# UniBwTAS/continuous_clustering

Measured on AMD Instinct MI355X. Metric: Mpoints/s clustered (64-beam streams), higher is better.
Workload: dtype f32

## Files before the change

continuous_clustering_amd/csrc/cc_device.h:

```cpp
#pragma once
#include <stdint.h>
#include <hip/hip_runtime.h>

#include "../../include/cc_hip.h"

namespace ccd
{

constexpr int WAVE = 64;
constexpr int MAX_ROWS_PER_LANE = 2;
constexpr int LINK_SLOTS = 4;
constexpr int WIN_COLS = 32;
constexpr int PP_SKIP = 0x7fffffff;
#ifndef CC_INS_WIN
#define CC_INS_WIN 64
#endif
constexpr int INS_WIN = CC_INS_WIN;
constexpr int SG_NAN = 1, SG_FOG = 2, SG_EGO = 4, SG_INCL_IGNORE = 8, SG_TOO_CLOSE = 16, SG_PENDING = 32;
constexpr unsigned NAN_RANGE_BITS = 0x7fc00001u;
#ifndef CC_TREE_SLOTS
#define CC_TREE_SLOTS 256
#endif
constexpr int TREE_SLOTS = CC_TREE_SLOTS;
#ifndef CC_TABLE_WAVES
// ... 27 lines not shown
    double finish_lower_bound;
    double last_round_min_az;
    int64_t clear_allowed;
    struct BatchDesc
    {
        int64_t seg_begin;
        int64_t seg_end;
        int64_t acp_next;
        int64_t pub_begin;
        int64_t pub_end;
        int64_t mode;
        int64_t fused;
    } batch[4];
    int32_t assoc_mode;
    int32_t pad1;
    int64_t cursor;
    int64_t pre_seg_begin;
    uint64_t firings_consumed;
    uint64_t cells_published;
    uint64_t clusters_finished;
    uint64_t exceed_one_rotation;
    uint64_t serial_columns;
    uint64_t stamp_alias_rounds;
    uint64_t batch_columns;
    uint64_t batch_bails;
    uint64_t batch_bail_reason[8];
    int64_t par_clear_done;
    int32_t par_bad;
    int32_t par_upto;
    int64_t serial_until;
    uint64_t dbg[16];
    int32_t error;
    int32_t n_events;
    int64_t error_a;
    int64_t error_b;
    int32_t n_links;
    int32_t pad2;
    int64_t overrun_col;
};

struct Planes
{
    float* dist;
    float* incaz;
    uint16_t* gtag;
    uint32_t* src;
    uint8_t* inten;
    int32_t* trig;
    int64_t* colg;
    double* colminaz;
    uint8_t* ground;
    uint8_t* debug;
    uint8_t* ignored;
    int32_t* root;
    uint32_t* id;
    double* t_fin;
    uint32_t* t_width;
    uint32_t* t_pts;
    int32_t* t_uf;
    uint32_t* t_cid;
    int32_t* t_pos;
    uint8_t* t_finished;
    int32_t* ulist;
    int32_t* ucomp;
    unsigned long long* agg_fin;
    long long* agg_min;
    long long* agg_max;
    uint32_t* agg_pts;
    uint32_t* agg_cid;
    int32_t* agg_first;
    uint8_t* agg_flag;
    cc_event* events;
    float* pp_x;
    float* pp_y;
    float* pp_z;
    float* pp_dist;
    float* pp_incl;
    float* pp_incaz;
    int32_t* pp_cir;
    float* sg_x2;
    float* sg_uz;
    uint8_t* sg_flags;
    float* sg_w;
    float4* sc_rec;
    int16_t* sc_parent;
    int16_t* sc_term;
    double* col_newfin;
    int32_t* col_info;
    unsigned* pk_meta;
    double* pk_fin;
    unsigned long long* pk_lk;
    uint16_t* col_act;
    uint8_t* sc_nlinks;
    unsigned long long* sc_links;
    double* sc_fin;
    uint16_t* sc_visits;
    int2* link_log;
    void* sl_rec;
    int32_t* sl_ctl;
    int32_t* sl_cols;
    int32_t* par_off;
    float* curtab;
    unsigned long long* tab_acc;
    float* tabc;
};

// ... 25 lines not shown
```

continuous_clustering_amd/csrc/cc_engine.hip:

```cpp
#include <hip/hip_runtime.h>

#include <algorithm>
#include <chrono>
#include <cstdlib>
#include <cmath>
#include <cstdio>
#include <cstring>
#include <functional>
#include <limits>
#include <mutex>
#include <string>
#include <vector>

#include "cc_kernels.h"

#ifndef CC_LWAVE_MAX_STREAMS
#define CC_LWAVE_MAX_STREAMS 256
#endif

using namespace ccd;

struct cc_engine
{
    int device{0};
// ... 263 lines not shown
    e->d_gather = nullptr;
    e->gather_bytes = 0;
    e->d_take_cursor = nullptr;
    e->d_take_plan = nullptr;
    e->d_take_ctl = nullptr;
    e->d_take_counts = nullptr;
    e->take_counts_cap = 0;
    e->d_tc_cursor = nullptr;
    e->d_tc_plan = nullptr;
    e->d_tc_table = nullptr;
    e->d_tc_ctl = nullptr;
    e->d_tc_slots = nullptr;
    e->tc_slots_cap = 0;
    e->d_small = nullptr;
    e->d_small_seq = nullptr;
    e->d_input_sum = nullptr;
    e->small_view_ok = false;
    e->small_seq_expected = 0;
    free_pinned(e, PIN_SHAPE);
    return CC_OK;
}

int allocate(cc_engine* e)
{
    const Geometry& g = e->g;
    const size_t S = (size_t) g.num_streams;
    const size_t C = S * (size_t) g.cells;
    const size_t L = S * (size_t) g.ring_cols;
    const size_t T = S * (size_t) g.tree_capacity;
    Planes& P = e->P;
    int rc = CC_OK;
    e->slab_planning = getenv("CC_NO_SLAB") == nullptr;
    e->slab_bytes = 0;
    e->slab_plan.clear();
#define A(field, count)                                \
    if ((rc = alloc_plane(e, &P.field, (count))) != 0) \
        return rc;
    A(dist, C) A(incaz, C) A(gtag, C) A(src, C) A(inten, C);
    A(trig, L) A(colg, L) A(colminaz, L);
    A(ground, C) A(debug, C) A(ignored, C) A(root, C) A(id, C);
    A(t_fin, C) A(t_width, C) A(t_pts, C) A(t_uf, C) A(t_cid, C) A(t_pos, C) A(t_finished, C);
    A(ulist, T) A(ucomp, T) A(agg_fin, T) A(agg_min, T) A(agg_max, T) A(agg_pts, T) A(agg_cid, T) A(agg_first, T) A(agg_flag, T);
    A(events, S * (size_t) g.event_capacity);
    A(sc_parent, C) A(sc_nlinks, C) A(sc_links, C) A(sc_fin, C);
    A(sc_term, C) A(col_newfin, L) A(col_info, L) A(col_act, L) A(pk_meta, C) A(pk_fin, C) A(pk_lk, C);
    A(sg_x2, C) A(sg_uz, C) A(sg_w, C) A(sg_flags, C) A(sc_rec, C);
    A(curtab, S * (size_t) g.num_rows);
    A(tab_acc, S * (size_t) g.tab_tiles * (size_t) g.num_rows);
    A(par_off, S * (size_t) cck::IP_MAXF);
    A(tabc, (size_t) BATCH_SLOTS * S * (size_t) g.tab_tiles * (size_t) g.num_rows);
    A(sc_visits, C);
    A(link_log, S * (size_t) g.link_capacity);
    A(sl_ctl, S * 4) A(sl_cols, L);
    if ((rc = alloc_plane(e, (unsigned long long**) &P.sl_rec, S * (size_t) cck::SL_CAP * sizeof(cck::ScanLongRec) / sizeof(unsigned long long))) != 0)
        return rc;
#undef A
    if ((rc = alloc_plane(e, &e->d_states, S)) != 0)
        return rc;
    if ((rc = alloc_plane(e, &e->d_par_left, 16)) != 0)
        return rc;
    if ((rc = alloc_plane(e, &e->d_bail_count, 4)) != 0)
        return rc;
    if ((rc = alloc_plane(e, &e->d_remaining, 1)) != 0)
        return rc;
    const bool slab = e->slab_planning;
    if (e->slab_planning)
    {
        e->slab_planning = false;
        char* base = nullptr;
        if ((rc = alloc_plane(e, &base, e->slab_bytes)) != 0)
            return rc;
        for (auto& f : e->slab_plan)
            *f.first = base + f.second;
        e->slab_plan.clear();
    }
    (void) slab;
    CC_HIP_CHECK(e, hipMemset(e->d_bail_count, 0, 4 * sizeof(int)));
    CC_HIP_CHECK(e, hipMemset(e->d_par_left, 0, 16 * sizeof(int)));
    CC_HIP_CHECK(e, hipMemset(e->d_remaining, 0, sizeof(int)));
    return CC_OK;
}

void fresh_stream_state(const cc_engine* e, StreamState* out)
{
    StreamState& st = *out;
    memset(&st, 0, sizeof(st));
    st.prev_rearmost = 0;
    st.prev_foremost = -1;
    st.first_unfinished = -1;
    st.ring_start = -1;
    st.ring_end = -1;
    st.first_column = -1;
    st.clear_done = -1;
    st.first_unpublished = -1;
    st.cluster_counter = 1;
    st.min_required = 0;
    st.finish_lower_bound = std::numeric_limits<double>::max();
    st.last_round_min_az = -1.0;
    st.overrun_col = std::numeric_limits<int64_t>::max();
    st.n_links = 0;
    for (auto& d : st.batch)
        d.seg_begin = d.seg_end = d.acp_next = d.pub_begin = d.pub_end = -1, d.mode = 0, d.fused = 0;
    st.assoc_mode = e->cfg.max_steps_in_row > WIN_COLS - 2 ? 1 : 0;
}

int reset_state(cc_engine* e, bool keep_table)
{
    e->small_view_ok = false;
    e->widest_steps_in_row = e->cfg.max_steps_in_row;
    std::fill(e->state_cached.begin(), e->state_cached.end(), 0);
    const Geometry& g = e->g;
    const size_t S = (size_t) g.num_streams;
    const size_t C = S * (size_t) g.cells;
    Planes& P = e->P;
    CC_HIP_CHECK(e, hipMemsetAsync(P.dist, 0xFF, C * sizeof(float), e->stream));
    CC_HIP_CHECK(e, hipMemsetAsync(P.gtag, 0, C * sizeof(uint16_t), e->stream));
    CC_HIP_CHECK(e, hipMemsetAsync(P.id, 0, C * sizeof(uint32_t), e->stream));
    CC_HIP_CHECK(e, hipMemsetAsync(P.ground, CC_GP_UNKNOWN, C, e->stream));
    CC_HIP_CHECK(e, hipMemsetAsync(P.debug, CC_DBG_WHITE, C, e->stream));
    CC_HIP_CHECK(e, hipMemsetAsync(P.ignored, 0, C, e->stream));
    CC_HIP_CHECK(e, hipMemsetAsync(P.root, 0xFF, C * sizeof(int32_t), e->stream));
    CC_HIP_CHECK(e, hipMemsetAsync(P.tab_acc, 0, S * (size_t) g.tab_tiles * (size_t) g.num_rows * sizeof(unsigned long long), e->stream));
    CC_HIP_CHECK(e, hipMemsetAsync(P.sl_ctl, 0, S * 4 * sizeof(int32_t), e->stream));
    if (!keep_table)
        CC_HIP_CHECK(e, hipMemsetAsync(P.curtab, 0xFF, S * (size_t) g.num_rows * sizeof(float), e->stream));
    std::vector<StreamState> init(S);
    for (auto& st : init)
        fresh_stream_state(e, &st);
    CC_HIP_CHECK(e, hipMemcpyAsync(e->d_states, init.data(), S * sizeof(StreamState), hipMemcpyHostToDevice, e->stream));
    if (e->d_take_cursor)
        CC_HIP_CHECK(e, hipMemsetAsync(e->d_take_cursor, 0, 2 * S * sizeof(long long), e->stream));
    if (e->d_tc_cursor)
        CC_HIP_CHECK(e, hipMemsetAsync(e->d_tc_cursor, 0, 2 * S * sizeof(long long), e->stream));
    CC_HIP_CHECK(e, hipStreamSynchronize(e->stream));
    for (auto& v : e->pending_events)
        v.clear();
    for (auto& v : e->pending_links)
        v.clear();
    e->batch_open = false;
    for (bool& b : e->assoc_pending)
        b = false;
    e->deferred_tail = nullptr;
    e->lazy_pending = false;
    e->lazy_prev_left = nullptr;
    e->lazy_miss = 0;
    e->lazy_clean = 0;
    e->lazy_ok = true;
    return CC_OK;
}

int reset_streams_state(cc_engine* e, const std::vector<int>& list)
{
    const Geometry& g = e->g;
    const Planes& P = e->P;
    const unsigned long long cells = (unsigned long long) g.cells;
    cck::ResetJob job;
    memset(&job, 0, sizeof(job));
    const cck::ResetFill fills[cck::RESET_PLANES] = {
        {(char*) P.dist, cells * sizeof(float), 0xFF, 0},
        {(char*) P.gtag, cells * sizeof(uint16_t), 0, 0},
        {(char*) P.id, cells * sizeof(uint32_t), 0, 0},
        {(char*) P.ground, cells, CC_GP_UNKNOWN, 0},
        {(char*) P.debug, cells, CC_DBG_WHITE, 0},
        {(char*) P.ignored, cells, 0, 0},
        {(char*) P.root, cells * sizeof(int32_t), 0xFF, 0},
        {(char*) P.tab_acc, (unsigned long long) g.tab_tiles * (unsigned long long) g.num_rows * sizeof(unsigned long long), 0, 0},
        {(char*) P.sl_ctl, 4 * sizeof(int32_t), 0, 0},
    };
    unsigned long long longest = 0;
    for (int k = 0; k < cck::RESET_PLANES; k++)
    {
        job.fill[k] = fills[k];
        longest = std::max(longest, fills[k].bytes);
    }
    fresh_stream_state(e, &job.fresh);
    job.states = e->d_states;
    job.take_cursor = e->d_take_cursor;
    job.tc_cursor = e->d_tc_cursor;
    job.num_streams = g.num_streams;
    int rc = ensure_gather(e, list.size() * sizeof(int));
    if (rc)
        return rc;
    CC_HIP_CHECK(e, hipMemcpyAsync(e->d_gather, list.data(), list.size() * sizeof(int), hipMemcpyHostToDevice, e->stream));
    constexpr size_t MAX_GRID_Y = 65535;
    for (size_t first = 0; first < list.size(); first += MAX_GRID_Y)
    {
        const size_t rows = std::min(MAX_GRID_Y, list.size() - first);
        const unsigned long long want = (longest + cck::RESET_CHUNK_BYTES - 1) / cck::RESET_CHUNK_BYTES;
        const unsigned chunks = (unsigned) std::max<unsigned long long>(1, std::min<unsigned long long>(want, (unsigned long long) cck::RESET_MAX_BLOCKS / rows));
        hipLaunchKernelGGL(cck::k_reset_streams, dim3(chunks, (unsigned) rows), dim3(cck::RESET_THREADS), 0, e->stream, job, (const int*) e->d_gather + first);
    }
    CC_HIP_CHECK(e, hipGetLastError());
    CC_HIP_CHECK(e, hipStreamSynchronize(e->stream));
    for (int s : list)
    {
        e->state_cached[s] = 0;
        if (s == e->small_view_stream)
            e->small_view_ok = false;
        e->pending_events[s].clear();
        e->pending_links[s].clear();
    }
    return CC_OK;
}

int ensure_prep(cc_engine* e, size_t points)
{
    if (e->prep_capacity >= points)
        return CC_OK;
    int rc;
    for (auto& q : e->pp)
        if ((rc = alloc_plane(e, &q.x, points)) || (rc = alloc_plane(e, &q.y, points)) || (rc = alloc_plane(e, &q.z, points)) ||
            (rc = alloc_plane(e, &q.dist, points)) || (rc = alloc_plane(e, &q.incl, points)) ||
            (rc = alloc_plane(e, &q.incaz, points)) || (rc = alloc_plane(e, &q.cir, points)))
            return rc;
    e->prep_capacity = points;
    e->small_graphs_stale = true;
    return CC_OK;
// ... 1949 lines not shown
```

continuous_clustering_amd/csrc/cc_k_base.h:

```cpp
#pragma once

#define CC_PI_F 3.14159274101257324219f
#define CC_2PI_D 6.283185307179586

__device__ __forceinline__ int lane_id()
{
    return threadIdx.x & 63;
}

__device__ __forceinline__ int f2i_x86(float v)
{
    if (!(v > -2147483904.0f && v < 2147483648.0f))
        return (int) 0x80000000;
    return (int) v;
}

template<int CTRL, int ROW_MASK>
__device__ __forceinline__ int dpp_mov_i32(int fill, int v)
{
    return __builtin_amdgcn_update_dpp(fill, v, CTRL, ROW_MASK, 0xf, false);
}
template<int CTRL, int ROW_MASK>
__device__ __forceinline__ long long dpp_mov_i64(long long fill, long long v)
{
// ... 257 lines not shown
}

constexpr uint16_t CELL_CLEARED = 0;
__device__ __forceinline__ uint16_t cell_tag(const long long pass)
{
    return (uint16_t) (0x8000u | ((unsigned) pass & 0x7fffu));
}

constexpr int IP_MAXF = 4608;

struct SP
{
    float *dist, *tabc;
    float* incaz;
    uint16_t* gtag;
    uint32_t* src;
    uint8_t *inten, *ground, *debug, *ignored;
    int32_t* trig;
    int64_t* colg;
    double* colminaz;
    int32_t* root;
    uint32_t* id;
    double* t_fin;
    uint32_t *t_width, *t_pts, *t_cid;
    int32_t *t_uf, *t_pos;
    uint8_t* t_finished;
    int32_t *ulist, *ucomp;
    unsigned long long* agg_fin;
    long long *agg_min, *agg_max;
    uint32_t *agg_pts, *agg_cid;
    int32_t* agg_first;
    uint8_t* agg_flag;
    float* curtab;
    unsigned long long* tab_acc;
    int32_t* par_off;
    cc_event* events;
    int16_t* sc_parent;
    int16_t* sc_term;
    double* col_newfin;
    int32_t* col_info;
    uint16_t* col_act;
    unsigned* pk_meta;
    double* pk_fin;
    unsigned long long* pk_lk;
    uint8_t* sc_nlinks;
    unsigned long long* sc_links;
    double* sc_fin;
    float *sg_x2, *sg_uz, *sg_w;
    uint8_t* sg_flags;
    float4* sc_rec;
    uint16_t* sc_visits;
    int2* link_log;
    int32_t* sl_cols;
};

__device__ __forceinline__ SP stream_ptrs(const Planes& P, const Geometry& g, int s)
{
    SP p;
    const size_t co = (size_t) s * (size_t) g.cells;
    const size_t lo = (size_t) s * (size_t) g.ring_cols;
    const size_t to = (size_t) s * (size_t) g.tree_capacity;
    p.dist = P.dist + co;
    p.incaz = P.incaz + co;
    p.gtag = P.gtag + co;
    p.src = P.src + co;
    p.inten = P.inten + co;
    p.ground = P.ground + co;
    p.debug = P.debug + co;
    p.ignored = P.ignored + co;
    p.trig = P.trig + lo;
    p.colg = P.colg + lo;
    p.colminaz = P.colminaz + lo;
    p.root = P.root + co;
    p.id = P.id + co;
    p.t_fin = P.t_fin + co;
    p.t_width = P.t_width + co;
    p.t_pts = P.t_pts + co;
    p.t_cid = P.t_cid + co;
    p.t_uf = P.t_uf + co;
    p.t_pos = P.t_pos + co;
    p.t_finished = P.t_finished + co;
    p.ulist = P.ulist + to;
    p.ucomp = P.ucomp + to;
    p.agg_fin = P.agg_fin + to;
    p.agg_min = P.agg_min + to;
    p.agg_max = P.agg_max + to;
    p.agg_pts = P.agg_pts + to;
    p.agg_cid = P.agg_cid + to;
    p.agg_first = P.agg_first + to;
    p.agg_flag = P.agg_flag + to;
    p.curtab = P.curtab + (size_t) s * g.num_rows;
    p.par_off = P.par_off + (size_t) s * IP_MAXF;
    p.tab_acc = P.tab_acc + (size_t) s * (size_t) g.tab_tiles * g.num_rows;
    p.tabc = P.tabc + (size_t) s * (size_t) g.tab_tiles * g.num_rows;
    p.events = P.events + (size_t) s * g.event_capacity;
    p.sc_parent = P.sc_parent + co;
    p.sc_term = P.sc_term + co;
    p.col_newfin = P.col_newfin + lo;
    p.col_info = P.col_info + lo;
    p.col_act = P.col_act + lo;
    p.pk_meta = P.pk_meta + co;
    p.pk_fin = P.pk_fin + co;
    p.pk_lk = P.pk_lk + co;
    p.sc_nlinks = P.sc_nlinks + co;
    p.sc_links = P.sc_links + co;
    p.sc_fin = P.sc_fin + co;
    p.sg_x2 = P.sg_x2 + co;
    p.sg_uz = P.sg_uz + co;
    p.sg_w = P.sg_w + co;
    p.sg_flags = P.sg_flags + co;
    p.sc_rec = P.sc_rec + co;
    p.sc_visits = P.sc_visits + co;
    p.link_log = P.link_log + (size_t) s * (size_t) g.link_capacity;
    p.sl_cols = P.sl_cols + lo;
    return p;
}

__device__ __forceinline__ double cell_fin(const cc_config& cfg, const SP& p, const int ci, const CazBase& cb)
{
    if (p.ignored[ci])
        return 0.;
    const float mad = ccm::asinf_exact(cfg.max_distance / p.dist[ci]);
    return cell_caz(cb, p.incaz[ci]) + (double) mad;
}
__device__ __forceinline__ double cell_fin_of(const Geometry& g, const cc_config& cfg, const SP& p, const int ci, const CazBase& cb)
{
    return g.scan_stores_fin ? p.sc_fin[ci] : cell_fin(cfg, p, ci, cb);
}
```

continuous_clustering_amd/csrc/cc_k_reset.h:

```cpp
#pragma once

constexpr int RESET_PLANES = 9;
constexpr int RESET_THREADS = 256;
constexpr unsigned long long RESET_CHUNK_BYTES = 16384;
constexpr int RESET_MAX_BLOCKS = 2048;
static_assert(sizeof(StreamState) % sizeof(unsigned long long) == 0 && alignof(StreamState) == alignof(unsigned long long), "the state is copied in 8-byte words");

struct ResetFill
{
    char* plane;
    unsigned long long bytes;
    unsigned value;
    unsigned pad;
};

struct ResetJob
{
    ResetFill fill[RESET_PLANES];
    StreamState fresh;
    StreamState* states;
    long long* take_cursor;
    long long* tc_cursor;
    int num_streams;
    int pad;
};

__device__ __forceinline__ void fill_slice(char* p, const unsigned long long bytes, const unsigned value, const unsigned chunk, const unsigned chunks)
{
    const unsigned long long to_boundary = (16ull - ((unsigned long long) p & 15ull)) & 15ull;
    const unsigned long long head = to_boundary < bytes ? to_boundary : bytes;
    const unsigned long long words = (bytes - head) >> 4;
    const unsigned long long tail = bytes - head - (words << 4);
    const unsigned w = (value & 0xffu) * 0x01010101u;
    const uint4 v = make_uint4(w, w, w, w);
    uint4* mid = (uint4*) (p + head);
    for (unsigned long long i = (unsigned long long) chunk * RESET_THREADS + threadIdx.x; i < words; i += (unsigned long long) chunks * RESET_THREADS)
        mid[i] = v;
    if (chunk == 0 && threadIdx.x < head)
        p[threadIdx.x] = (char) value;
    if (chunk == chunks - 1 && threadIdx.x < tail)
        p[head + (words << 4) + threadIdx.x] = (char) value;
}

__global__ __launch_bounds__(RESET_THREADS) void k_reset_streams(const ResetJob job, const int* __restrict__ list)
{
    const int s = list[blockIdx.y];
    if (s < 0 || s >= job.num_streams)
        return;
    for (int k = 0; k < RESET_PLANES; k++)
        fill_slice(job.fill[k].plane + (unsigned long long) s * job.fill[k].bytes, job.fill[k].bytes, job.fill[k].value, blockIdx.x, gridDim.x);
    if (blockIdx.x != 0)
        return;
    const unsigned long long* src = (const unsigned long long*) &job.fresh;
    unsigned long long* dst = (unsigned long long*) &job.states[s];
    for (unsigned i = threadIdx.x; i < sizeof(StreamState) / sizeof(unsigned long long); i += RESET_THREADS)
// ... 10 lines not shown
```

continuous_clustering_amd/csrc/cc_k_scan.h:

```cpp
#pragma once

#ifndef CC_SCAN_BLOCKS
#define CC_SCAN_BLOCKS 256
#endif
constexpr int SCAN_BLOCKS = CC_SCAN_BLOCKS;

template<int RPL, bool MIRROR>
__device__ __forceinline__ void scan_body(const Geometry& g, const cc_config& cfg, const Planes& P, StreamState* states, int first_stream, int slot,
                                          const int bx, const int by, const int ny)
{
    const int s = first_stream + bx;
    const int lane = lane_id();
    const StreamState* st = &states[s];
    if (st->error != 0 || st->batch[slot].seg_begin < 0 || st->batch[slot].mode != 0)
        return;
    AssocCtx c;
    c.p = stream_ptrs(P, g, s);
    const SP& p = c.p;
    const int R = c.R = g.num_rows;
    c.NC = g.num_columns;
    const int RC = c.RC = g.ring_cols;
    c.az_width = g.az_width;
    c.maxd2 = g.max_distance_squared;
    c.max_steps_in_row = cfg.max_steps_in_row;
// ... 294 lines not shown
            continue;
        P.pp_x[i] = q.x;
        P.pp_y[i] = q.y;
        P.pp_z[i] = q.z;
        P.pp_dist[i] = q.dist;
        P.pp_incl[i] = q.incl;
        P.pp_incaz[i] = q.incaz;
    }
    if (threadIdx.x == 0)
    {
        long long* w = insert2_sync_words<1>(R);
        lds_st(w, 0ll);
        lds_st(w + 1, 0ll);
        lds_st(w + 2, -1ll);
    }
    __syncthreads();
    SF_MARK(1)
    if (threadIdx.x < 128)
        insert2_body<1, true, true>(g, cfg, P, states, stream, slot, inten, n, remaining, n, 0, 0);
    __syncthreads();
    SF_MARK(2)
    if (threadIdx.x < 64)
        seg_small_body(g, cfg, P, states, stream, slot, poses, n, 0, ego, n, 0);
    __syncthreads();
    SF_MARK(3)
    if (g.mirror_fields)
        scan_body<1, true>(g, cfg, P, states, stream, slot, 0, uniform_i32((int) (threadIdx.x >> 6)), 4);
    else
        scan_body<1, false>(g, cfg, P, states, stream, slot, 0, uniform_i32((int) (threadIdx.x >> 6)), 4);
#ifdef CC_SF_STATS
    __syncthreads();
    SF_MARK(4)
    if (threadIdx.x == 0)
    {
        for (int i = 0; i < 4; i++)
            st->dbg[i] += sf_t[i + 1] - sf_t[i];
        st->dbg[4] += 1;
    }
#endif
}

#ifndef CC_SCAN_TILE_CELLS
#define CC_SCAN_TILE_CELLS 256
#endif
constexpr int SCAN_TILE_CELLS = CC_SCAN_TILE_CELLS;

struct ScanCfg
{
    int R, RC, max_col_steps, stop_min;
    bool stop_enabled;
    float maxd2;
};

struct ScanPoint
{
    float4 me;
    float mad;
    int row, needed, bound;
    int sb, down, d, oc, orow;
    int rooted, parent, nlinks, overflow, visits, reach;
    unsigned long long packed;
    bool run;

    __device__ __forceinline__ void next_column(const ScanCfg& c)
    {
        if ((rooted && c.stop_enabled && sb >= c.stop_min) || oc == bound || sb + 1 > needed)
            run = false;
        else
        {
            sb++;
            oc = oc == 0 ? c.RC - 1 : oc - 1;
            down = 0;
            d = 0;
            orow = row;
        }
    }
    __device__ __forceinline__ void next_direction(const ScanCfg& c)
    {
        if (down == 0 && sb > 0)
        {
            down = 1;
            d = 1;
            orow = row + 1;
            if (!(orow < c.R && d <= c.max_col_steps))
                next_column(c);
        }
        else
            next_column(c);
    }
    __device__ __forceinline__ void start(const ScanCfg& c, const bool have, const int lc)
    {
        sb = 0, down = 0, d = 1, oc = lc, orow = row - 1;
        rooted = 0, parent = -1, nlinks = 0, overflow = 0, visits = 0, reach = 0;
        packed = 0;
        run = have;
        if (run && !(orow >= 0 && d <= c.max_col_steps))
            next_direction(c);
    }
    template<bool MIRROR>
    __device__ __forceinline__ void step(const ScanCfg& c, const SP& p)
    {
        const float4 o = p.sc_rec[oc * c.R + orow];
        const unsigned char oign = p.ignored[oc * c.R + orow];
        if (MIRROR)
        {
            visits++;
            reach = sb;
        }
        if (ccm::absf(o.w - me.w) > mad)
            next_direction(c);
        else
        {
            const float dx = me.x - o.x, dy = me.y - o.y, dz = me.z - o.z;
            if (!oign && dx * dx + dy * dy + dz * dz < c.maxd2)
            {
                const int cand = (sb << 8) | orow;
                if (!rooted)
                    parent = cand;
                else if (nlinks < LINK_SLOTS)
                {
                    packed |= (unsigned long long) cand << (16 * nlinks);
                    nlinks++;
                }
                else
                    overflow = 1;
                rooted = 1;
            }
            if (rooted && c.stop_enabled && d >= c.stop_min)
                next_direction(c);
            else
            {
                d++;
                orow = down ? orow + 1 : orow - 1;
                if (!(orow >= 0 && orow < c.R && d <= c.max_col_steps))
                    next_direction(c);
            }
        }
    }
};

constexpr int SL_CAP = 8192;
struct ScanLongRec
{
    int ci;
    int oc;
    short orow, sb, d, needed;
    short parent;
    unsigned char down, rooted, nlinks, flags;
    float mad;
    unsigned long long packed;
};
static_assert(sizeof(ScanLongRec) == 40, "long-scan record");

#ifndef CC_SCAN_CAP
#define CC_SCAN_CAP 6
#endif
constexpr int SCAN_CAP = CC_SCAN_CAP;

template<int RPL, bool MIRROR, bool SPLIT = false>
__global__ __launch_bounds__(64) void k_scan2(Geometry g, cc_config cfg, Planes P, StreamState* states, int first_stream, int slot)
{
    static_assert(!(SPLIT && MIRROR), "the long-scan list does not carry the mirror's visit counts");
    const int s = first_stream + blockIdx.x;
    const int lane = lane_id();
    const StreamState* st = &states[s];
    if (st->error != 0 || st->batch[slot].seg_begin < 0 || st->batch[slot].mode != 0)
        return;
    const SP p = stream_ptrs(P, g, s);
    const int R = g.num_rows, RC = g.ring_cols;
    ScanCfg sc;
    sc.R = R, sc.RC = RC;
    sc.maxd2 = g.max_distance_squared;
    sc.max_col_steps = cfg.max_steps_in_column;
    sc.stop_enabled = cfg.stop_after_association_enabled != 0;
    sc.stop_min = cfg.stop_after_association_min_steps;
    const int max_row_steps = cfg.max_steps_in_row;
    const int TC = SCAN_TILE_CELLS / (RPL * 64);
    __shared__ unsigned short s_list[SCAN_TILE_CELLS];
    __shared__ short s_parent[SCAN_TILE_CELLS];
    __shared__ unsigned char s_nlinks[SCAN_TILE_CELLS];
    __shared__ unsigned short s_visits[MIRROR ? SCAN_TILE_CELLS : 1];
    __shared__ unsigned char s_reach[MIRROR ? SCAN_TILE_CELLS : 1];
    __shared__ double s_fin[SCAN_TILE_CELLS];
    __shared__ unsigned long long s_links[SCAN_TILE_CELLS];
    int* const sl_ctl = P.sl_ctl + (size_t) s * 4;
    ScanLongRec* const sl_rec = (ScanLongRec*) P.sl_rec + (size_t) s * SL_CAP;
    const long long col_begin = st->batch[slot].acp_next, col_end = st->batch[slot].seg_end, first_column = st->first_column;
    const int first_lc = (int) (first_column % RC);
    const long long n_tiles = (col_end - col_begin + TC - 1) / TC;
    for (long long tile = blockIdx.y; tile < n_tiles; tile += gridDim.y)
    {
        const long long gc0 = col_begin + tile * TC;
        const int ncols = (int) (col_end - gc0 < TC ? col_end - gc0 : TC);
        const int lc0 = (int) (gc0 % RC);
        const long long rot0 = gc0 / g.num_columns;
        const int cir0 = (int) (gc0 - rot0 * g.num_columns);
        int n_act = 0;
        for (int j = 0; j < TC * RPL; j++)
        {
            const int tc = j / RPL, row = (j % RPL) * 64 + lane;
            const int tl = tc * RPL * 64 + row;
            bool act = false;
            if (tc < ncols && row < R)
            {
                int lc = lc0 + tc;
                lc = lc >= RC ? lc - RC : lc;
                act = p.ignored[lc * R + row] == 0;
            }
            s_parent[tl] = -2;
            s_nlinks[tl] = 0;
            s_fin[tl] = 0.;
            s_links[tl] = 0;
            if (MIRROR)
            {
                s_visits[tl] = 0;
                s_reach[tl] = 0;
            }
            const unsigned long long m = __ballot(act);
            if (act)
                s_list[n_act + __popcll(m & lanes_below())] = (unsigned short) tl;
            n_act += __popcll(m);
        }
        wave_lds_fence();
        unsigned deferred = 0;
        for (int base = 0; base < n_act; base += 64)
        {
            const bool have = base + lane < n_act;
            const int tl = have ? (int) s_list[base + lane] : 0;
            const int tc = tl / (RPL * 64), row = tl % (RPL * 64);
            const long long gc = gc0 + tc;
            int lc = lc0 + tc;
            lc = lc >= RC ? lc - RC : lc;
            const int ci = lc * R + row;
            ScanPoint q;
            q.me = make_float4(0.f, 0.f, 0.f, 0.f);
            q.mad = 0.f;
            q.row = row;
            double fin = 0.;
            q.needed = -1;
            if (have)
            {
                q.me = p.sc_rec[ci];
                q.mad = ccm::asinf_exact(cfg.max_distance / p.dist[ci]);
                fin = cell_caz(caz_base_of_rotation(rot0 + (cir0 + tc >= g.num_columns ? 1 : 0)), p.incaz[ci]) + (double) q.mad;
                q.needed = f2i_x86(__builtin_ceilf(q.mad / g.az_width));
                q.needed = q.needed < max_row_steps ? q.needed : max_row_steps;
            }
            q.bound = (gc - first_column) <= (long long) max_row_steps + 1 ? first_lc : -1;
            q.start(sc, have, lc);
            bool pending = false;
            if (SPLIT)
            {
                for (int it = 0; it < g.scan_cap && __any(q.run); it++)
                    if (q.run)
                        q.template step<false>(sc, p);
                const unsigned long long m = __ballot(q.run);
                if (m)
                {
                    int lbase = 0;
                    if (lane == (int) __ffsll((long long) m) - 1)
                        lbase = atomicAdd(&sl_ctl[0], (int) __popcll(m));
                    lbase = __shfl(lbase, (int) __ffsll((long long) m) - 1);
                    const int idx = lbase + (int) __popcll(m & lanes_below());
                    if (q.run && idx < g.sl_cap)
                    {
                        ScanLongRec r;
                        r.ci = ci, r.oc = q.oc;
                        r.orow = (short) q.orow, r.sb = (short) q.sb, r.d = (short) q.d, r.needed = (short) q.needed;
                        r.parent = (short) q.parent;
                        r.down = (unsigned char) q.down, r.rooted = (unsigned char) q.rooted, r.nlinks = (unsigned char) q.nlinks;
                        r.flags = (unsigned char) ((q.overflow ? 1 : 0) | (q.bound >= 0 ? 2 : 0));
                        r.mad = q.mad;
                        r.packed = q.packed;
                        sl_rec[idx] = r;
                        pending = true;
                        q.run = false;
                    }
                    while (__any(q.run))
                        if (q.run)
                            q.template step<false>(sc, p);
                }
                for (int t2 = 0; t2 < TC; t2++)
                    if (__any(pending && tc == t2))
                        deferred |= 1u << t2;
            }
            else
            {
                while (__any(q.run))
                    if (q.run)
                        q.template step<MIRROR>(sc, p);
            }
            if (have)
            {
                s_parent[tl] = (short) (pending ? -3 : q.parent);
                s_nlinks[tl] = (unsigned char) (q.overflow ? 255 : q.nlinks);
                s_fin[tl] = fin;
                s_links[tl] = q.packed;
                if (MIRROR)
                {
                    s_visits[tl] = sat_u16(q.visits);
                    s_reach[tl] = (unsigned char) q.reach;
                }
            }
        }
        wave_lds_fence();
        for (int tc = 0; tc < ncols; tc++)
        {
            int lc = lc0 + tc;
            lc = lc >= RC ? lc - RC : lc;
            int parent[RPL], nlinks[RPL];
            double fin[RPL];
            unsigned long long packed[RPL];
            int reach = 0;
            const bool later = SPLIT && ((deferred >> tc) & 1u) != 0;
#pragma unroll
            for (int k = 0; k < RPL; k++)
            {
                const int row = k * 64 + lane;
                const int tl = tc * RPL * 64 + row;
                parent[k] = s_parent[tl];
                nlinks[k] = s_nlinks[tl];
                fin[k] = s_fin[tl];
                packed[k] = s_links[tl];
                if (MIRROR)
                    reach = (int) s_reach[tl] > reach ? (int) s_reach[tl] : reach;
                if (row < R)
                {
                    const int ci = lc * R + row;
                    if (g.scan_stores_fin)
                        p.sc_fin[ci] = fin[k];
                    if (!(later && parent[k] == -3))
                    {
                        p.sc_parent[ci] = (int16_t) parent[k];
                        p.sc_nlinks[ci] = (uint8_t) nlinks[k];
                        if (nlinks[k] > 0)
                            p.sc_links[ci] = packed[k];
                    }
                    if (MIRROR)
                        p.sc_visits[ci] = s_visits[tl];
                }
            }
            if (later)
            {
                if (lane == 0)
                    p.sl_cols[atomicAdd(&sl_ctl[2], 1)] = lc;
            }
            else
                scan_column_epilogue<RPL, MIRROR>(p, R, lc, lane, parent, nlinks, fin, packed, reach);
        }
        wave_lds_fence();
    }
}

#ifndef CC_SCAN_LONG_BLOCKS
#define CC_SCAN_LONG_BLOCKS 16
#endif
constexpr int SCAN_LONG_BLOCKS = CC_SCAN_LONG_BLOCKS;
constexpr int SCAN_EPI_BLOCKS = 16;

template<int RPL>
__global__ __launch_bounds__(64) void k_scan2_long(Geometry g, cc_config cfg, Planes P, StreamState* states, int first_stream, int slot, int* __restrict__ stat)
{
    const int s = first_stream + blockIdx.x;
    int* const sl_ctl = P.sl_ctl + (size_t) s * 4;
    int n = sl_ctl[0];
    if (n <= 0)
        return;
    n = n < g.sl_cap ? n : g.sl_cap;
    const StreamState* st = &states[s];
    const int lane = lane_id();
    const SP p = stream_ptrs(P, g, s);
    const ScanLongRec* const sl_rec = (ScanLongRec*) P.sl_rec + (size_t) s * SL_CAP;
    const int R = g.num_rows, RC = g.ring_cols;
    ScanCfg sc;
    sc.R = R, sc.RC = RC;
    sc.maxd2 = g.max_distance_squared;
    sc.max_col_steps = cfg.max_steps_in_column;
    sc.stop_enabled = cfg.stop_after_association_enabled != 0;
    sc.stop_min = cfg.stop_after_association_min_steps;
    const int first_lc = (int) (st->first_column % RC);
    ScanPoint q;
    q.run = false;
    q.me = make_float4(0.f, 0.f, 0.f, 0.f);
    q.mad = 0.f, q.row = 0, q.needed = 0, q.bound = -1, q.sb = 0, q.down = 0, q.d = 0, q.oc = 0, q.orow = 0;
    q.rooted = 0, q.parent = -1, q.nlinks = 0, q.overflow = 0, q.visits = 0, q.reach = 0, q.packed = 0ull;
    int ci = 0;
    int nvis = 0;
    bool more = true;
    for (;;)
    {
        const unsigned long long idle = __ballot(!q.run);
        if (more && idle)
        {
            int lbase = 0;
            if (lane == (int) __ffsll((long long) idle) - 1)
                lbase = atomicAdd(&sl_ctl[1], (int) __popcll(idle));
            lbase = __shfl(lbase, (int) __ffsll((long long) idle) - 1);
            const int idx = lbase + (int) __popcll(idle & lanes_below());
            if (!q.run && idx < n)
            {
                const ScanLongRec r = sl_rec[idx];
                ci = r.ci;
                q.me = p.sc_rec[ci];
                q.mad = r.mad;
                q.row = ci % R;
                q.needed = r.needed;
                q.bound = (r.flags & 2) ? first_lc : -1;
                q.sb = r.sb, q.down = r.down, q.d = r.d, q.oc = r.oc, q.orow = r.orow;
                q.rooted = r.rooted, q.parent = r.parent, q.nlinks = r.nlinks, q.overflow = r.flags & 1;
                q.packed = r.packed;
                q.run = true;
            }
            more = lbase + (int) __popcll(idle) < n;
        }
        if (!__any(q.run))
            break;
        for (int it = 0; it < 8; it++)
            if (q.run)
            {
                q.template step<false>(sc, p);
                nvis++;
                if (!q.run)
                {
                    p.sc_parent[ci] = (int16_t) q.parent;
                    p.sc_nlinks[ci] = (uint8_t) (q.overflow ? 255 : q.nlinks);
                    if (q.nlinks > 0)
                        p.sc_links[ci] = q.packed;
                }
            }
    }
    if (stat)
    {
        for (int off = 32; off > 0; off >>= 1)
            nvis += __shfl_down(nvis, off, 64);
        if (lane == 0 && nvis > 0)
            atomicAdd(&stat[1], nvis);
    }
}

template<int RPL>
__global__ __launch_bounds__(64) void k_scan2_epi(Geometry g, cc_config cfg, Planes P, StreamState* states, int first_stream, int slot, int* __restrict__ stat)
{
    const int s = first_stream + blockIdx.x;
    int* const sl_ctl = P.sl_ctl + (size_t) s * 4;
    const int nd = sl_ctl[2];
    const int lane = lane_id();
    if (stat && blockIdx.y == 0 && lane == 0)
    {
        const StreamState* st = &states[s];
        if (st->error == 0 && st->batch[slot].seg_begin >= 0 && st->batch[slot].mode == 0)
        {
            atomicAdd(&stat[2], (int) (st->batch[slot].seg_end - st->batch[slot].acp_next));
        }
    }
    if (nd <= 0 && sl_ctl[0] <= 0)
        return;
    const SP p = stream_ptrs(P, g, s);
    const int R = g.num_rows;
    for (int i = blockIdx.y; i < nd; i += gridDim.y)
    {
        const int lc = p.sl_cols[i];
        const CazBase cb = caz_base_of_column(p.colg[lc], g.num_columns);
        int parent[RPL], nlinks[RPL];
        double fin[RPL];
        unsigned long long packed[RPL];
#pragma unroll
        for (int k = 0; k < RPL; k++)
        {
            const int row = k * 64 + lane;
            parent[k] = -2, nlinks[k] = 0, fin[k] = 0., packed[k] = 0ull;
            if (row < R)
            {
                const int ci = lc * R + row;
// ... 19 lines not shown
```

continuous_clustering_amd/csrc/cc_k_segment.h:

```cpp
#pragma once


template<int RPL>
__device__ __forceinline__ void table_scan_tiles(const SP& p, const int R, const int ntiles, const int lane)
{
    float carry[RPL];
#pragma unroll
    for (int k = 0; k < RPL; k++)
    {
        const int row = k * 64 + lane;
        carry[k] = row < R ? p.curtab[row] : 0.f;
    }
    constexpr int U = 8;
    for (int t0 = 0; t0 < ntiles; t0 += U)
    {
        float v[U][RPL];
#pragma unroll
        for (int u = 0; u < U; u++)
#pragma unroll
            for (int k = 0; k < RPL; k++)
            {
                const int row = k * 64 + lane;
                v[u][k] = (row < R && t0 + u < ntiles) ? p.tabc[(size_t) (t0 + u) * R + row] : __builtin_nanf("");
            }
// ... 746 lines not shown
                            nf0 |= f << (8 * u);
                        else
                            nf1 |= f << (8 * (u - 4));
                    }
                }
            };
            int b = R - 8;
            load_chunk(b);
            for (; b > -8; b -= 8)
            {
                float x8[8], z8[8], w8[8];
#pragma unroll
                for (int u = 0; u < 8; u++)
                {
                    x8[u] = nx[u];
                    z8[u] = nz[u];
                    w8[u] = nw[u];
                }
                const unsigned f0 = nf0, f1 = nf1;
                if (b - 8 > -8)
                    load_chunk(b - 8);
#pragma unroll
                for (int u = 0; u < 8; u++)
                    if (b + u >= 0)
                        x2[(b + u) & (SEG_X2_RING - 1)] = x8[u];
                auto x2_below = [&](const int below, const bool wanted) -> float
                {
                    float v = x2[below & (SEG_X2_RING - 1)];
                    const bool deep = wanted & (below >= b + SEG_X2_RING);
                    if (__any(deep))
                        if (deep)
                            v = gx[below];
                    return v;
                };
#pragma unroll
                for (int u = 7; u >= 0; u--)
                {
                    const int row = b + u;
                    if (row < 0)
                        break;
                    float tab_u = 0.f;
                    const bool pend = row_all(row, (int) (((u < 4 ? f0 : f1) >> (8 * (u & 3))) & 0xffu), x8[u], z8[u], w8[u], tab_in[row], x2_below,
                                              [&](const float tab) { tab_u = tab; });
                    if (__any(pend))
                        if (pend && ccm::atan2f_exact(cfg.max_distance, w8[u]) < tab_u)
                            oo[row] |= 0x80;
                }
            }
        }
    }
    __syncthreads();
    {
        int lc = lc0;
        for (int c = 0; c < ncols; c++)
        {
            for (int row = lane; row < R; row += 64)
            {
                const size_t ci = (size_t) lc * R + row;
                const unsigned char o = l_out[c * PB + row];
                constexpr unsigned long long GV = (unsigned long long) CC_GP_UNKNOWN | ((unsigned long long) CC_GP_GROUND << 8) |
                                                  ((unsigned long long) CC_GP_OBSTACLE << 16) | ((unsigned long long) CC_GP_EGO_VEHICLE << 24) |
                                                  ((unsigned long long) CC_GP_FOG << 32);
                constexpr unsigned long long DV0 = (unsigned long long) CC_DBG_WHITE | ((unsigned long long) CC_DBG_GRAY << 8) |
                                                   ((unsigned long long) CC_DBG_ORANGE << 16) | ((unsigned long long) CC_DBG_GREEN << 24) |
                                                   ((unsigned long long) CC_DBG_YELLOWGREEN << 32) | ((unsigned long long) CC_DBG_YELLOW << 40) |
                                                   ((unsigned long long) CC_DBG_RED << 48) | ((unsigned long long) CC_DBG_DARKRED << 56);
                constexpr unsigned DV1 = (unsigned) CC_DBG_VIOLET | ((unsigned) CC_DBG_LIGHTGRAY << 8);
                const unsigned dcode = (o >> 3) & 15;
                p.ground[ci] = (unsigned char) (GV >> (8 * (o & 7)));
                p.debug[ci] = (unsigned char) (dcode < 8 ? (DV0 >> (8 * dcode)) : (unsigned long long) (DV1 >> (8 * (dcode - 8))));
                const bool ign = (o & 7) != SG_G_OBSTACLE || (o & 0x80);
                p.ignored[ci] = ign ? 1 : 0;
            }
            lc = lc + 1 == RC ? 0 : lc + 1;
        }
    }
}

__device__ __forceinline__ void seg_small_body(const Geometry& g, const cc_config& cfg, const Planes& P, StreamState* states, int first_stream, int slot,
                                               const double* __restrict__ poses, long long n_total, long long fbase, const double* __restrict__ ego,
                                               long long n_batch, const int sl)
{
    const int s = first_stream + sl;
    StreamState* st = &states[s];
    const int lane = lane_id();
    if (lane == 0)
        st->batch[slot].mode = st->assoc_mode;
    const long long seg_begin = st->batch[slot].seg_begin, seg_end = st->batch[slot].seg_end;
    if (seg_begin < 0 || seg_begin >= seg_end || st->error != 0)
        return;
    if (!st->has_robot_tf)
    {
        if (lane == 0)
            raise_error(st, CC_ERR_NO_ROBOT_TRANSFORM, seg_begin, 0);
        return;
    }
    const SP p = stream_ptrs(P, g, s);
    const int R = g.num_rows, RC = g.ring_cols, NC = g.num_columns;
    const int row = lane;
    const bool inrow = row < R;
    const float height_sensor_to_ground = -(float) st->robot_from_sensor[11] + cfg.height_ref_to_ground_;
    const bool supplement = cfg.supplement_inclination_angle_for_nan_cells != 0;
    const bool step_filter = cfg.ignore_points_with_too_big_inclination_angle_diff != 0;
    const bool no_terrain = cfg.use_terrain == 0;
    const unsigned long long le = lane == 63 ? ~0ull : ((2ull << lane) - 1ull);
    const unsigned long long below = ~le, above = le >> 1;
    float tabrow = inrow ? p.curtab[row] : 0.f;
    int lc = (int) (seg_begin % RC);
    long long rot = seg_begin / NC;
    int cir = (int) (seg_begin - rot * NC);
    long long pass = seg_begin / RC;
    CazBase cb = caz_base_of_rotation(rot);
    for (long long gc = seg_begin; gc < seg_end; gc++)
    {
        const size_t ci = (size_t) lc * R + row;
        const uint16_t tag = cell_tag(pass);
        float cx[1] = {0.f}, cy[1] = {0.f}, cz[1] = {0.f}, dist[1] = {__builtin_nanf("")}, incl[1] = {__builtin_nanf("")};
        uint8_t inten[1] = {0};
        float incaz = 0.f;
        bool empty_cell = false, overrun = false;
        long long overrun_gcol = -1;
        if (inrow)
        {
            const uint16_t tg = p.gtag[ci];
            dist[0] = p.dist[ci];
            if (tg == tag)
            {
// ... 88 lines not shown
            const bool has_lg = ml != 0;
            const int lgrow = has_lg ? __ffsll((long long) ml) - 1 : lane;
            const float lgx = __shfl(cur2x, lgrow, 64), lgy = __shfl(cur2y, lgrow, 64);
            const float lg2x = has_lg ? lgx : 0.f, lgz = has_lg ? lgy : height_sensor_to_ground;
            const float l2cx = cur2x - lg2x, l2cy = cur2y - lgz;
            const float slope_to_lg = l2cy / l2cx;
            const bool flat_lg = (ccm::absf(slope_to_lg) < cfg.max_slope) & (l2cx > 0);
            const bool green = !fod & flat_prev;
            const bool yellowgreen = !green & no_terrain & fod & flat_prev & flat_lg;
            const bool yellow = !green & !yellowgreen & no_terrain & (ccm::absf(l2cx) < cfg.ground_because_close_to_last_certain_ground_max_dist_diff) &
                                (ccm::absf(l2cy) < cfg.ground_because_close_to_last_certain_ground_max_z_diff);
            const unsigned dn = normal ? (green ? (unsigned) SG_D_GREEN
                                                : (yellowgreen ? (unsigned) SG_D_YELLOWGREEN : (yellow ? (unsigned) SG_D_YELLOW : (unsigned) SG_D_RED)))
                                       : d;
            const bool changed = dn != d;
            d = dn;
            if (!__any(changed))
                break;
        }
        unsigned gl = (d == (unsigned) SG_D_ORANGE || d == (unsigned) SG_D_RED) ? (unsigned) SG_G_OBSTACLE : (unsigned) SG_G_GROUND;
        gl = valid ? gl : (unsigned) SG_G_UNKNOWN;
        if (f & SG_EGO)
        {
            gl = SG_G_EGO;
            d = SG_D_VIOLET;
        }
        if (f & SG_FOG)
        {
            gl = SG_G_FOG;
            d = SG_D_LIGHTGRAY;
        }
        if ((f & SG_NAN) || !inrow)
        {
            gl = SG_G_UNKNOWN;
            d = SG_D_WHITE;
        }
        {
            const unsigned long long REDm = __ballot(normal & (d == (unsigned) SG_D_RED));
            const unsigned long long RA = REDm & above;
            const bool has_ra = RA != 0;
            const int ra = has_ra ? 63 - __clzll((long long) RA) : lane;
            const float xr = __shfl(cur2x, ra, 64);
            const bool pass_test = has_ra & ((d == (unsigned) SG_D_YELLOW) |
                                             ((gl == (unsigned) SG_G_GROUND) & (ccm::absf(xr - cur2x) < cfg.obstacle_because_next_certain_obstacle_max_dist_diff)));
            const unsigned long long NP = __ballot(!pass_test);
            const unsigned long long le_ra = ra == 63 ? ~0ull : ((2ull << ra) - 1ull);
            const bool reached = has_ra & ((NP & le & ~le_ra) == 0);
            if (reached & (gl == (unsigned) SG_G_GROUND))
            {
                gl = SG_G_OBSTACLE;
                d = SG_D_DARKRED;
            }
        }
        if (inrow)
        {
            constexpr unsigned long long GV = (unsigned long long) CC_GP_UNKNOWN | ((unsigned long long) CC_GP_GROUND << 8) |
                                              ((unsigned long long) CC_GP_OBSTACLE << 16) | ((unsigned long long) CC_GP_EGO_VEHICLE << 24) |
                                              ((unsigned long long) CC_GP_FOG << 32);
            constexpr unsigned long long DV0 = (unsigned long long) CC_DBG_WHITE | ((unsigned long long) CC_DBG_GRAY << 8) |
                                               ((unsigned long long) CC_DBG_ORANGE << 16) | ((unsigned long long) CC_DBG_GREEN << 24) |
                                               ((unsigned long long) CC_DBG_YELLOWGREEN << 32) | ((unsigned long long) CC_DBG_YELLOW << 40) |
                                               ((unsigned long long) CC_DBG_RED << 48) | ((unsigned long long) CC_DBG_DARKRED << 56);
            constexpr unsigned DV1 = (unsigned) CC_DBG_VIOLET | ((unsigned) CC_DBG_LIGHTGRAY << 8);
            p.ground[ci] = (unsigned char) (GV >> (8 * gl));
            p.debug[ci] = (unsigned char) (d < 8 ? (DV0 >> (8 * d)) : (unsigned long long) (DV1 >> (8 * (d - 8))));
            p.ignored[ci] = (gl != (unsigned) SG_G_OBSTACLE || ign) ? 1 : 0;
            if (empty_cell)
                p.gtag[ci] = tag;
            if (is_nan)
                p.sc_rec[ci].w = sincl;
        }
        int kpos = 0x7fffffff, kneg = 0x7fffffff;
        if (inrow && !is_nan)
            caz_key(incaz, kpos, kneg);
        const double min_az = column_min_caz(cb, kpos, kneg, inrow && is_nan, gc, g.az_width);
        if (lane == 0)
        {
            p.colg[lc] = gc;
            p.colminaz[lc] = min_az;
        }
        lc = lc + 1 == RC ? 0 : lc + 1;
        pass += lc == 0 ? 1 : 0;
        cir = cir + 1 == NC ? 0 : cir + 1;
        if (cir == 0)
        {
            rot++;
            cb = caz_base_of_rotation(rot);
        }
    }
    if (inrow)
        p.curtab[row] = tabrow;
}

__global__ __launch_bounds__(64) void k_seg_small(Geometry g, cc_config cfg, Planes P, StreamState* states, int first_stream, int slot,
                                                  const double* __restrict__ poses, long long n_total, long long fbase, const double* __restrict__ ego,
                                                  long long n_batch)
{
    seg_small_body(g, cfg, P, states, first_stream, slot, poses, n_total, fbase, ego, n_batch, (int) blockIdx.x);
}
```

Before: 19980.

## Maintain per-column scannable bitmask and stage it in LDS for tile scans

Segmentation kernels now also write a per-column 64-bit ballot mask of scannable (non-ignored obstacle) rows into a new scan_mask plane. The tiled scan kernel loads the masks for its tile window into shared memory and tests neighbour activity and ignored state from LDS bits instead of per-cell byte loads from global memory. This cuts scattered global reads during neighbour scans, at the cost of an extra plane, extra writes and resets, and an early return when max_steps_in_row exceeds the window. The small-body mask write indexes by lc alone and ignores the row-word stride, which looks fragile when there is more than one word per column.

```diff
diff --git a/continuous_clustering_amd/csrc/cc_device.h b/continuous_clustering_amd/csrc/cc_device.h
--- a/continuous_clustering_amd/csrc/cc_device.h
+++ b/continuous_clustering_amd/csrc/cc_device.h
@@ -103,6 +103,7 @@
     uint8_t* ground;
     uint8_t* debug;
     uint8_t* ignored;
+    unsigned long long* scan_mask;
     int32_t* root;
     uint32_t* id;
     double* t_fin;
diff --git a/continuous_clustering_amd/csrc/cc_engine.hip b/continuous_clustering_amd/csrc/cc_engine.hip
--- a/continuous_clustering_amd/csrc/cc_engine.hip
+++ b/continuous_clustering_amd/csrc/cc_engine.hip
@@ -339,6 +339,7 @@
     A(sc_visits, C);
     A(link_log, S * (size_t) g.link_capacity);
     A(sl_ctl, S * 4) A(sl_cols, L);
+    A(scan_mask, L * (size_t) ((g.num_rows + 63) / 64));
     if ((rc = alloc_plane(e, (unsigned long long**) &P.sl_rec, S * (size_t) cck::SL_CAP * sizeof(cck::ScanLongRec) / sizeof(unsigned long long))) != 0)
         return rc;
 #undef A
@@ -406,6 +407,7 @@
     CC_HIP_CHECK(e, hipMemsetAsync(P.ground, CC_GP_UNKNOWN, C, e->stream));
     CC_HIP_CHECK(e, hipMemsetAsync(P.debug, CC_DBG_WHITE, C, e->stream));
     CC_HIP_CHECK(e, hipMemsetAsync(P.ignored, 0, C, e->stream));
+    CC_HIP_CHECK(e, hipMemsetAsync(P.scan_mask, 0, S * (size_t) g.ring_cols * (size_t) ((g.num_rows + 63) / 64) * sizeof(unsigned long long), e->stream));
     CC_HIP_CHECK(e, hipMemsetAsync(P.root, 0xFF, C * sizeof(int32_t), e->stream));
     CC_HIP_CHECK(e, hipMemsetAsync(P.tab_acc, 0, S * (size_t) g.tab_tiles * (size_t) g.num_rows * sizeof(unsigned long long), e->stream));
     CC_HIP_CHECK(e, hipMemsetAsync(P.sl_ctl, 0, S * 4 * sizeof(int32_t), e->stream));
@@ -450,6 +452,7 @@
         {(char*) P.ground, cells, CC_GP_UNKNOWN, 0},
         {(char*) P.debug, cells, CC_DBG_WHITE, 0},
         {(char*) P.ignored, cells, 0, 0},
+        {(char*) P.scan_mask, (unsigned long long) g.ring_cols * (unsigned long long) ((g.num_rows + 63) / 64) * sizeof(unsigned long long), 0, 0},
         {(char*) P.root, cells * sizeof(int32_t), 0xFF, 0},
         {(char*) P.tab_acc, (unsigned long long) g.tab_tiles * (unsigned long long) g.num_rows * sizeof(unsigned long long), 0, 0},
         {(char*) P.sl_ctl, 4 * sizeof(int32_t), 0, 0},
diff --git a/continuous_clustering_amd/csrc/cc_k_base.h b/continuous_clustering_amd/csrc/cc_k_base.h
--- a/continuous_clustering_amd/csrc/cc_k_base.h
+++ b/continuous_clustering_amd/csrc/cc_k_base.h
@@ -333,6 +333,7 @@
     uint16_t* sc_visits;
     int2* link_log;
     int32_t* sl_cols;
+    unsigned long long* scan_mask;
 };
 
 __device__ __forceinline__ SP stream_ptrs(const Planes& P, const Geometry& g, int s)
@@ -394,6 +395,7 @@
     p.sc_visits = P.sc_visits + co;
     p.link_log = P.link_log + (size_t) s * (size_t) g.link_capacity;
     p.sl_cols = P.sl_cols + lo;
+    p.scan_mask = P.scan_mask + lo * (size_t) ((g.num_rows + 63) / 64);
     return p;
 }
 
diff --git a/continuous_clustering_amd/csrc/cc_k_reset.h b/continuous_clustering_amd/csrc/cc_k_reset.h
--- a/continuous_clustering_amd/csrc/cc_k_reset.h
+++ b/continuous_clustering_amd/csrc/cc_k_reset.h
@@ -1,6 +1,6 @@
 #pragma once
 
-constexpr int RESET_PLANES = 9;
+constexpr int RESET_PLANES = 10;
 constexpr int RESET_THREADS = 256;
 constexpr unsigned long long RESET_CHUNK_BYTES = 16384;
 constexpr int RESET_MAX_BLOCKS = 2048;
diff --git a/continuous_clustering_amd/csrc/cc_k_scan.h b/continuous_clustering_amd/csrc/cc_k_scan.h
--- a/continuous_clustering_amd/csrc/cc_k_scan.h
+++ b/continuous_clustering_amd/csrc/cc_k_scan.h
@@ -370,6 +370,30 @@
     float maxd2;
 };
 
+struct IgnoredPlane
+{
+    const uint8_t* ignored;
+    int R;
+    __device__ __forceinline__ bool operator()(const int oc, const int orow) const
+    {
+        return ignored[oc * R + orow] != 0;
+    }
+};
+constexpr int SCAN_MASK_COLS = 64;
+template<int RPL>
+struct IgnoredMask
+{
+    const unsigned long long* mask;
+    int lc_last, RC;
+    __device__ __forceinline__ bool operator()(const int oc, const int orow) const
+    {
+        int j = lc_last - oc;
+        j = j < 0 ? j + RC : j;
+        const unsigned long long w = mask[RPL == 1 ? j : j * RPL + (orow >> 6)];
+        return ((w >> (orow & 63)) & 1ull) == 0;
+    }
+};
+
 struct ScanPoint
 {
     float4 me;
@@ -415,11 +439,11 @@
         if (run && !(orow >= 0 && d <= c.max_col_steps))
             next_direction(c);
     }
-    template<bool MIRROR>
-    __device__ __forceinline__ void step(const ScanCfg& c, const SP& p)
+    template<bool MIRROR, class IGN>
+    __device__ __forceinline__ void step(const ScanCfg& c, const SP& p, const IGN& ign)
     {
         const float4 o = p.sc_rec[oc * c.R + orow];
-        const unsigned char oign = p.ignored[oc * c.R + orow];
+        const bool oign = ign(oc, orow);
         if (MIRROR)
         {
             visits++;
@@ -494,6 +518,11 @@
     sc.stop_min = cfg.stop_after_association_min_steps;
     const int max_row_steps = cfg.max_steps_in_row;
     const int TC = SCAN_TILE_CELLS / (RPL * 64);
+    if (max_row_steps > WIN_COLS - 2)
+        return;
+    static_assert(SCAN_TILE_CELLS / 64 + WIN_COLS - 2 + 1 < SCAN_MASK_COLS, "the masks of a tile's window fit s_mask");
+    const int W = (R + 63) >> 6;
+    __shared__ unsigned long long s_mask[SCAN_MASK_COLS * RPL];
     __shared__ unsigned short s_list[SCAN_TILE_CELLS];
     __shared__ short s_parent[SCAN_TILE_CELLS];
     __shared__ unsigned char s_nlinks[SCAN_TILE_CELLS];
@@ -513,18 +542,27 @@
         const int lc0 = (int) (gc0 % RC);
         const long long rot0 = gc0 / g.num_columns;
         const int cir0 = (int) (gc0 - rot0 * g.num_columns);
+        int lc_last = lc0 + ncols - 1;
+        lc_last = lc_last >= RC ? lc_last - RC : lc_last;
+        if (lane <= ncols + max_row_steps)
+        {
+            int c = lc_last - lane;
+            c = c < 0 ? c + RC : c;
+            c = c < 0 ? 0 : c;
+#pragma unroll
+            for (int k = 0; k < RPL; k++)
+                s_mask[lane * RPL + k] = k < W ? p.scan_mask[(size_t) c * W + k] : 0ull;
+        }
+        wave_lds_fence();
+        const IgnoredMask<RPL> ign_mask{s_mask, lc_last, RC};
         int n_act = 0;
         for (int j = 0; j < TC * RPL; j++)
         {
             const int tc = j / RPL, row = (j % RPL) * 64 + lane;
             const int tl = tc * RPL * 64 + row;
             bool act = false;
-            if (tc < ncols && row < R)
-            {
-                int lc = lc0 + tc;
-                lc = lc >= RC ? lc - RC : lc;
-                act = p.ignored[lc * R + row] == 0;
-            }
+            if (tc < ncols)
+                act = ((s_mask[(ncols - 1 - tc) * RPL + j % RPL] >> lane) & 1ull) != 0;
             s_parent[tl] = -2;
             s_nlinks[tl] = 0;
             s_fin[tl] = 0.;
@@ -571,7 +609,7 @@
             {
                 for (int it = 0; it < g.scan_cap && __any(q.run); it++)
                     if (q.run)
-                        q.template step<false>(sc, p);
+                        q.template step<false>(sc, p, ign_mask);
                 const unsigned long long m = __ballot(q.run);
                 if (m)
                 {
@@ -596,7 +634,7 @@
                     }
                     while (__any(q.run))
                         if (q.run)
-                            q.template step<false>(sc, p);
+                            q.template step<false>(sc, p, ign_mask);
                 }
                 for (int t2 = 0; t2 < TC; t2++)
                     if (__any(pending && tc == t2))
@@ -606,7 +644,7 @@
             {
                 while (__any(q.run))
                     if (q.run)
-                        q.template step<MIRROR>(sc, p);
+                        q.template step<MIRROR>(sc, p, ign_mask);
             }
             if (have)
             {
@@ -697,6 +735,7 @@
     sc.stop_enabled = cfg.stop_after_association_enabled != 0;
     sc.stop_min = cfg.stop_after_association_min_steps;
     const int first_lc = (int) (st->first_column % RC);
+    const IgnoredPlane ign_plane{p.ignored, R};
     ScanPoint q;
     q.run = false;
     q.me = make_float4(0.f, 0.f, 0.f, 0.f);
@@ -736,7 +775,7 @@
         for (int it = 0; it < 8; it++)
             if (q.run)
             {
-                q.template step<false>(sc, p);
+                q.template step<false>(sc, p, ign_plane);
                 nvis++;
                 if (!q.run)
                 {
diff --git a/continuous_clustering_amd/csrc/cc_k_segment.h b/continuous_clustering_amd/csrc/cc_k_segment.h
--- a/continuous_clustering_amd/csrc/cc_k_segment.h
+++ b/continuous_clustering_amd/csrc/cc_k_segment.h
@@ -822,27 +822,48 @@
     __syncthreads();
     {
         int lc = lc0;
+        const int W = (R + 63) >> 6;
+        unsigned long long mk0 = 0ull, mk1 = 0ull;
         for (int c = 0; c < ncols; c++)
         {
-            for (int row = lane; row < R; row += 64)
-            {
-                const size_t ci = (size_t) lc * R + row;
-                const unsigned char o = l_out[c * PB + row];
-                constexpr unsigned long long GV = (unsigned long long) CC_GP_UNKNOWN | ((unsigned long long) CC_GP_GROUND << 8) |
-                                                  ((unsigned long long) CC_GP_OBSTACLE << 16) | ((unsigned long long) CC_GP_EGO_VEHICLE << 24) |
-                                                  ((unsigned long long) CC_GP_FOG << 32);
-                constexpr unsigned long long DV0 = (unsigned long long) CC_DBG_WHITE | ((unsigned long long) CC_DBG_GRAY << 8) |
-                                                   ((unsigned long long) CC_DBG_ORANGE << 16) | ((unsigned long long) CC_DBG_GREEN << 24) |
-                                                   ((unsigned long long) CC_DBG_YELLOWGREEN << 32) | ((unsigned long long) CC_DBG_YELLOW << 40) |
-                                                   ((unsigned long long) CC_DBG_RED << 48) | ((unsigned long long) CC_DBG_DARKRED << 56);
-                constexpr unsigned DV1 = (unsigned) CC_DBG_VIOLET | ((unsigned) CC_DBG_LIGHTGRAY << 8);
-                const unsigned dcode = (o >> 3) & 15;
-                p.ground[ci] = (unsigned char) (GV >> (8 * (o & 7)));
-                p.debug[ci] = (unsigned char) (dcode < 8 ? (DV0 >> (8 * dcode)) : (unsigned long long) (DV1 >> (8 * (dcode - 8))));
-                const bool ign = (o & 7) != SG_G_OBSTACLE || (o & 0x80);
-                p.ignored[ci] = ign ? 1 : 0;
+            for (int k = 0; k < W; k++)
+            {
+                const int row = k * 64 + lane;
+                bool scannable = false;
+                if (row < R)
+                {
+                    const size_t ci = (size_t) lc * R + row;
+                    const unsigned char o = l_out[c * PB + row];
+                    constexpr unsigned long long GV = (unsigned long long) CC_GP_UNKNOWN | ((unsigned long long) CC_GP_GROUND << 8) |
+                                                      ((unsigned long long) CC_GP_OBSTACLE << 16) | ((unsigned long long) CC_GP_EGO_VEHICLE << 24) |
+                                                      ((unsigned long long) CC_GP_FOG << 32);
+                    constexpr unsigned long long DV0 = (unsigned long long) CC_DBG_WHITE | ((unsigned long long) CC_DBG_GRAY << 8) |
+                                                       ((unsigned long long) CC_DBG_ORANGE << 16) | ((unsigned long long) CC_DBG_GREEN << 24) |
+                                                       ((unsigned long long) CC_DBG_YELLOWGREEN << 32) | ((unsigned long long) CC_DBG_YELLOW << 40) |
+                                                       ((unsigned long long) CC_DBG_RED << 48) | ((unsigned long long) CC_DBG_DARKRED << 56);
+                    constexpr unsigned DV1 = (unsigned) CC_DBG_VIOLET | ((unsigned) CC_DBG_LIGHTGRAY << 8);
+                    const unsigned dcode = (o >> 3) & 15;
+                    p.ground[ci] = (unsigned char) (GV >> (8 * (o & 7)));
+                    p.debug[ci] = (unsigned char) (dcode < 8 ? (DV0 >> (8 * dcode)) : (unsigned long long) (DV1 >> (8 * (dcode - 8))));
+                    const bool ign = (o & 7) != SG_G_OBSTACLE || (o & 0x80);
+                    p.ignored[ci] = ign ? 1 : 0;
+                    scannable = !ign;
+                }
+                const unsigned long long m = __ballot(scannable);
+                if (k == 0)
+                    mk0 = lane == c ? m : mk0;
+                else
+                    mk1 = lane == c ? m : mk1;
             }
             lc = lc + 1 == RC ? 0 : lc + 1;
+        }
+        if (lane < ncols)
+        {
+            int l = lc0 + lane;
+            l = l >= RC ? l - RC : l;
+            p.scan_mask[(size_t) l * W] = mk0;
+            if (W > 1)
+                p.scan_mask[(size_t) l * W + 1] = mk1;
         }
     }
 }
@@ -1037,6 +1058,11 @@
                 d = SG_D_DARKRED;
             }
         }
+        {
+            const unsigned long long m = __ballot(inrow && gl == (unsigned) SG_G_OBSTACLE && !ign);
+            if (lane == 0)
+                p.scan_mask[lc] = m;
+        }
         if (inrow)
         {
             constexpr unsigned long long GV = (unsigned long long) CC_GP_UNKNOWN | ((unsigned long long) CC_GP_GROUND << 8) |
```

Result: no change. 20220, median of 6 (+1.2%).
